# Ivordir/YALPS

Measured on AMD Instinct MI355X. Metric: fp64 pivots/sec on dense m x n tableau, higher is better.
Workload: dtype f64

## Files before the change

yalps_amd/csrc/common.cuh:

```cuda
#pragma once


constexpr int RUNNING = -1;
constexpr int SHARD_SWEEP_MISSING = 77;
constexpr int MODE_FUSED = 0, MODE_DECIDE = 1, MODE_APPLY = 2, MODE_SHARD = 3;
constexpr int SHARD_HDR = 8;
constexpr int MAX_SHARDS = 8;
constexpr int LAUNCHES_PER_GRAPH = 64;
constexpr int MAX_BLOCKS = 1024;
constexpr unsigned long long FLUSHED = 0x7FF8C0DEC0DE5EEDull;

struct alignas(16) YConst {
    int32_t height;
    int32_t check_cycles;
    int64_t hist_cap;
    int32_t *hist_leaving, *hist_entering;
    double precision, max_pivots;
};

struct alignas(16) YState {
    int32_t status;
    int32_t phase;
    int32_t bootstrap;
    int32_t la;
// ... 23 lines not shown
#ifndef YALPS_PANEL_SETS
#define YALPS_PANEL_SETS 1
#endif
constexpr int HP_SCAL = 8 + 2 * 16;
constexpr int STREAM3_MAXD = 16;
constexpr int STREAM3_PANEL_UNITS = 512;
__host__ __device__ constexpr int stream3_panel_units(int) { return STREAM3_PANEL_UNITS; }
constexpr int STREAM3_DEPTH_J16 = 16;
constexpr int DSHARD_MAXD = 16;
constexpr int DSHARD_PANEL_UNITS = 512;

struct alignas(16) Part {
    double key;
    int32_t idx;
    int32_t pad_;
};

struct Desc {
    double *mat[2];
    double *rhs[2];
    int32_t *pos, *var;
    YState *st;
    YConst *cst;
    Part *part_ratio[2];
    Part *part_rhs[2];
    int32_t w, n, pitch, hcap;
    int32_t nb;
    int32_t nshards, shard_rank, row_base;
    int32_t bounds[MAX_SHARDS + 1];
    double *rc_rows[2];
    double *rc_key[2];
    double *rc_tag[2];
    unsigned long long *rc_flag[2];
    int32_t *rc_err;
    unsigned long long *rc_verdict;
    unsigned long long *rc_rowflag;
    double *ob_park;
    int32_t *hp_xcc;
    unsigned long long *hp_flag;
    double *hp_scal;
    int32_t perm_len;
    int32_t extra;
    int32_t xl_ofs;
    double *gen_prow, *gen_scal;
    unsigned long long *sw_sync, *sw_recs;
    int32_t sw_nt;
    int32_t delay_depth;
    double *pend;
    double *obj[2];
    double *dpend, *dcolv, *dnqv, *dlav;
    DelayState *dstate;
    int32_t *cyc_verdict;
    int32_t ext_sweep;
    unsigned long long *dbg;
};
constexpr int STAMP_WORDS = 24;

struct KI {
    double k;
    int i;
};

__device__ __forceinline__ bool ki_better(double ka, int ia, double kb, int ib) {
    return ka < kb || (ka == kb && ia < ib);
}

constexpr int DPP_XOR1 = 0xB1, DPP_XOR2 = 0x4E, DPP_HALF_MIRROR = 0x141, DPP_MIRROR = 0x140;

template <int CTRL>
__device__ __forceinline__ int dpp_i32(int v) {
    return __builtin_amdgcn_update_dpp(v, v, CTRL, 0xF, 0xF, false);
}
template <int CTRL>
__device__ __forceinline__ double dpp_f64(double v) {
    const int lo = dpp_i32<CTRL>(__double2loint(v)), hi = dpp_i32<CTRL>(__double2hiint(v));
    return __hiloint2double(hi, lo);
}
__device__ __forceinline__ double row16_min(double v) {
    v = fmin(v, dpp_f64<DPP_XOR1>(v));
    v = fmin(v, dpp_f64<DPP_XOR2>(v));
    v = fmin(v, dpp_f64<DPP_HALF_MIRROR>(v));
    v = fmin(v, dpp_f64<DPP_MIRROR>(v));
    return v;
}
__device__ __forceinline__ int row16_min(int v) {
    v = min(v, dpp_i32<DPP_XOR1>(v));
    v = min(v, dpp_i32<DPP_XOR2>(v));
    v = min(v, dpp_i32<DPP_HALF_MIRROR>(v));
// ... 125 lines not shown
```

yalps_amd/csrc/resident2_kernel.cuh:

```cuda
#pragma once


__device__ __forceinline__ double min_f64_raw(double a, double b) {
    double r;
    asm("v_min_f64 %0, %1, %2" : "=v"(r) : "v"(a), "v"(b));
    return r;
}
constexpr int DPP_ROW_BCAST15 = 0x142, DPP_ROW_BCAST31 = 0x143;
template <int CTRL, int ROW_MASK>
__device__ __forceinline__ int dpp_i32_rm(int v) {
    return __builtin_amdgcn_update_dpp(v, v, CTRL, ROW_MASK, 0xF, false);
}
template <int CTRL, int ROW_MASK>
__device__ __forceinline__ double dpp_f64_rm(double v) {
    const int lo = dpp_i32_rm<CTRL, ROW_MASK>(__double2loint(v)), hi = dpp_i32_rm<CTRL, ROW_MASK>(__double2hiint(v));
    return __hiloint2double(hi, lo);
}
template <int STEPS>
__device__ __forceinline__ double rowN_min_raw(double v) {
    v = min_f64_raw(v, dpp_f64<DPP_XOR1>(v));
    if constexpr (STEPS >= 2) v = min_f64_raw(v, dpp_f64<DPP_XOR2>(v));
    if constexpr (STEPS >= 3) v = min_f64_raw(v, dpp_f64<DPP_HALF_MIRROR>(v));
    if constexpr (STEPS >= 4) v = min_f64_raw(v, dpp_f64<DPP_MIRROR>(v));
    return v;
// ... 14 lines not shown
    r.k = lane_f64(m, 63);
    const bool hit = v.k == r.k;
    const unsigned long long mask = __builtin_amdgcn_ballot_w64(hit);
    if (__popcll(mask) == 1) {
        r.i = __builtin_amdgcn_readlane(v.i, __ffsll((long long)mask) - 1);
    } else {
        int i = rowN_min<4>(hit ? v.i : INT_MAX);
        i = min(i, dpp_i32_rm<DPP_ROW_BCAST15, 0xA>(i));
        i = min(i, dpp_i32_rm<DPP_ROW_BCAST31, 0xC>(i));
        r.i = __builtin_amdgcn_readlane(i, 63);
    }
    return r;
}
template <int T>
__device__ __forceinline__ KI block_argmin2(KI v, double (*sk)[16], int (*si)[16], int slot) {
    constexpr int NW = T / 64, STEPS = NW == 16 ? 4 : NW == 8 ? 3 : NW == 4 ? 2 : 1;
    static_assert(NW == 2 || NW == 4 || NW == 8 || NW == 16, "waves per workgroup");
    v = wave_argmin2(v);
    const int lane = threadIdx.x & 63, wv = threadIdx.x >> 6;
    if (lane == 0) {
        sk[slot][wv] = v.k;
        si[slot][wv] = v.i;
    }
    __syncthreads();
    const double k = sk[slot][lane & (NW - 1)];
    const int i = si[slot][lane & (NW - 1)];
    const double km = rowN_min_raw<STEPS>(k);
    KI r;
    r.k = uniform_f64(km);
    r.i = __builtin_amdgcn_readfirstlane(rowN_min<STEPS>(k == km ? i : INT_MAX));
    return r;
}

template <int T, int J, int R>
__global__ __launch_bounds__(T) void resident2_kernel(Desc d, int parity, int chunk) {
    constexpr int SPLIT = YALPS_SPLIT_NUM * R / 4;
    constexpr unsigned FULL = (1u << (2 * J)) - 1u;
    __shared__ double sk[2][16];
    __shared__ int si[2][16];
    __shared__ double sh_cf[2][R + 2];
    __shared__ double sh_nq[R + 2];
    __shared__ double sh_raw[R + 2];
    __shared__ double sh_ck;
    __shared__ int sh_ci, sh_cg, sh_fail, sh_flag, sh_verdict, sh_pnz;
    extern __shared__ int sh_perm[];

    const int tid = threadIdx.x, NB = d.nb, b = blockIdx.x;
    const int wave = __builtin_amdgcn_readfirstlane(tid >> 6);
    const YState *Sin = d.st + parity;
    YState *Sout = d.st + (parity ^ 1);
    const YConst *C = d.cst;
    if (Sin->status != RUNNING) {
        if (b == 0 && tid == 0) state_copy(Sout, Sin);
        return;
    }
    const int h = C->height, n = d.n, pitch = d.pitch, w = d.w;
    const double precision = C->precision, max_pivots = C->max_pivots;
    const int mbuf = Sin->mbuf;
    const double *matA = d.mat[mbuf];
    const double *rhsA = d.rhs[mbuf];
    int phase = Sin->phase;
    double iter = Sin->iter;
    int64_t pivots = Sin->pivots;
    int64_t hist_len = Sin->hist_len;
    const bool check_cycles = C->check_cycles != 0;
    int slot = 0;

    int cofs[J];
#pragma unroll
    for (int j = 0; j < J; j++) {
        const int c0 = 2 * (tid + j * T);
        cofs[j] = c0 < pitch ? c0 : 0;
    }
    unsigned padmask = 0;
#pragma unroll
    for (int j = 0; j < J; j++)
#pragma unroll
        for (int k = 0; k < 2; k++)
            if (2 * (tid + j * T) + k >= n) padmask |= 1u << (2 * j + k);
    double2 x[R][J], o[J];
#pragma unroll
    for (int j = 0; j < J; j++) {
        o[j] = *reinterpret_cast<const double2 *>(matA + cofs[j]);
        if (padmask & (1u << (2 * j))) o[j].x = -INFINITY;
        if (padmask & (1u << (2 * j + 1))) o[j].y = -INFINITY;
    }
#pragma unroll
    for (int g = 0; g < R; g++) {
        const int r = b + NB * g;
        const double *mr = matA + (size_t)(r < h ? r : b) * pitch;
#pragma unroll
        for (int j = 0; j < J; j++) x[g][j] = *reinterpret_cast<const double2 *>(mr + cofs[j]);
    }
    const int my_r = b + NB * tid;
    const bool my_live = tid < R && my_r < h;
    double my_rhs = rhsA[my_live ? my_r : 0];
    if (b == 0) {
        for (int i = tid; i < d.perm_len; i += T) {
            sh_perm[i] = d.var[i];
            sh_perm[d.perm_len + i] = d.pos[i];
        }
    }
    if (tid == 0) sh_fail = 0;
    __syncthreads();

    int la = 0;
    double la_val = 0.0;
    unsigned epoch = 0;
    int cur = 0;
    auto price = [&]() __attribute__((always_inline)) {
        double best = precision;
        int bi = INT_MAX;
#pragma unroll
        for (int j = 0; j < J; j++) {
            const int c0 = 2 * (tid + j * T);
            if (o[j].x > best) {
                best = o[j].x;
                bi = c0 + 1;
            }
            if (o[j].y > best) {
                best = o[j].y;
                bi = c0 + 2;
            }
        }
        KI v = {bi == INT_MAX ? INFINITY : -best, bi};
        v = block_argmin2<T>(v, sk, si, slot);
        slot ^= 1;
        la = v.i == INT_MAX ? 0 : v.i;
        la_val = -v.k;
    };
    auto deposit_la = [&](const double2 (&pvn)[J], unsigned nzmask, bool pending) __attribute__((always_inline)) {
        const int ula = (la - 1) >> 1, ela = (la - 1) & 1, lt = ula % T, lj = ula / T;
        if (la > 0 && wave == (lt >> 6)) {
#pragma unroll
            for (int j = 0; j < J; j++)
#pragma unroll
                for (int e = 0; e < 2; e++)
                    if (2 * (tid + j * T) + e + 1 == la) {
#pragma unroll
                        for (int g = 0; g < R; g++) sh_raw[g] = e ? x[g][j].y : x[g][j].x;
                        if (pending) {
// ... 23 lines not shown
            }
            if (kind == 2 && tid < R) sh_cf[which][tid] = value;
            c = wave_argmin2(c);
            if (tid == 0) {
                sh_ck = c.k;
                sh_ci = c.i;
                sh_cg = c.i == INT_MAX ? 0 : c.i / NB;
            }
        }
        if (barrier) __syncthreads();
    };
    auto publish_flag = [&]() __attribute__((always_inline)) {
        const int par = epoch & 1;
        asm volatile("s_waitcnt vmcnt(0)" ::: "memory");
        __syncthreads();
        if (tid == 0)
            st16_sc1(reinterpret_cast<double *>(d.rc_flag[par] + 2 * b),
                     make_double2(sh_ck, __longlong_as_double((long long)(((unsigned long long)epoch << 32) | (unsigned)sh_ci))));
    };
    auto publish_stores = [&](int cg) __attribute__((always_inline)) {
        epoch++;
        double *dst = d.rc_rows[epoch & 1] + (size_t)b * pitch;
#pragma unroll
        for (int g = 0; g < R; g++) {
            if (g == cg) {
#pragma unroll
                for (int j = 0; j < J; j++) {
                    const int c0 = 2 * (tid + j * T);
                    if (c0 < pitch) st16_sc1(dst + c0, x[g][j]);
                }
            }
        }
        if (tid == cg) st_sc1(d.rc_key[epoch & 1] + b, my_rhs);
    };
    int done = 0, term = RUNNING;
    double term_result = NAN;
    bool stop = false;
#ifdef YALPS_STAMPS
    unsigned long long st_acc[20] = {}, st_last = 0, st_t0 = 0, st_r0 = 0;
#endif
    auto check = [&]() __attribute__((always_inline)) {
        if (done == chunk) {
            stop = true;
        } else if (!(iter < max_pivots)) {
            term = YALPS_CYCLED;
            stop = true;
        } else if (phase == 2 && la == 0) {
            term = YALPS_OPTIMAL;
            stop = true;
        }
    };
    const double2 no_row[J] = {};
    auto open_round = [&]() __attribute__((always_inline)) {
        double value = 0.0;
        if (phase == 2) {
            deposit_la(no_row, 0u, false);
            if (tid < R) value = sh_raw[tid];
        }
        candidate(phase, value, cur, true);
        publish_stores(__builtin_amdgcn_readfirstlane(sh_cg));
        publish_flag();
    };

    price();
    check();
    if (!stop) open_round();
#ifdef YALPS_STAMPS
    asm volatile("s_memtime %0\n\ts_memrealtime %1\n\ts_waitcnt lgkmcnt(0)" : "=s"(st_t0), "=s"(st_r0)::"memory");
    st_last = st_t0;
#endif
    while (!stop) {
        const int par = epoch & 1;
        KI c = {INFINITY, INT_MAX};
        if (tid < NB) {
            unsigned long long f = 0;
            unsigned spins = 0;
            [[maybe_unused]] unsigned long long spin_t0 = 0;
            double2 rec;
            for (;;) {
                rec = ld16_sc1_one(d.rc_flag[par] + 2 * tid);
                f = (unsigned long long)__double_as_longlong(rec.y);
                if ((unsigned)(f >> 32) == epoch) break;
                if (RESIDENT_SPIN_EXPIRED(spins, spin_t0, d.rc_err)) {
                    sh_fail = 1;
                    __hip_atomic_store(d.rc_err, 1, __ATOMIC_RELAXED, __HIP_MEMORY_SCOPE_AGENT);
                    break;
                }
                __builtin_amdgcn_s_sleep(2);
            }
            c.i = (int)(unsigned)f;
            c.k = rec.x;
#ifdef YALPS_AB_POLL_GUARD
            if (c.i != INT_MAX && (unsigned)c.i >= (unsigned)h) {
// ... 8 lines not shown
        YSTAMP(1);
        if (sh_fail) return;
        if (c.i == INT_MAX) {
            if (phase == 1) {
                phase = 2;
                iter = 0.0;
                hist_len = 0;
                check();
                if (!stop) open_round();
            } else {
                term = YALPS_UNBOUNDED;
                term_result = (double)la;
                stop = true;
            }
            YSTAMP(14);
            continue;
        }
#if defined(YALPS_AB_RETURN_GUARD) || defined(YALPS_AB_NOGUARD) || defined(YALPS_AB_POLL_GUARD)
        const int row = c.i, owner = row % NB;
#else
        const int row_in = c.i, row = (unsigned)row_in < (unsigned)h ? row_in : 0, owner = row % NB;
        if (row != row_in && tid == 0) __hip_atomic_store(d.rc_err, 1, __ATOMIC_RELAXED, __HIP_MEMORY_SCOPE_AGENT);
#endif
#ifdef YALPS_AB_RETURN_GUARD
        if ((unsigned)row >= (unsigned)h) {
            if (tid == 0) __hip_atomic_store(d.rc_err, 1, __ATOMIC_RELAXED, __HIP_MEMORY_SCOPE_AGENT);
            return;
        }
#endif
        const double *src = d.rc_rows[par] + (size_t)owner * pitch;
        double2 pv[J];
        const double rhs_row = ld_sc1(d.rc_key[par] + owner);
        double q = ld_sc1(src + (phase == 2 ? la - 1 : 0));
        ld16_sc1<J>(pv, src, cofs);
        YSTAMP(2);
        int col = la;
        double coef0 = la_val;
        if (phase == 1) {
            KI e = {INFINITY, INT_MAX};
#pragma unroll
            for (int j = 0; j < J; j++) {
                const int c0 = 2 * (tid + j * T);
#pragma unroll
                for (int k = 0; k < 2; k++) {
                    const double coefficient = elem(pv[j], k);
                    if (c0 + k < n && coefficient < -precision) {
                        const double ratio = -elem(o[j], k) / coefficient;
                        if (ratio > -INFINITY && ki_better(-ratio, c0 + k + 1, e.k, e.i)) {
                            e.k = -ratio;
                            e.i = c0 + k + 1;
                        }
                    }
                }
            }
            e = block_argmin2<T>(e, sk, si, slot);
            slot ^= 1;
            if (e.i == INT_MAX) {
                term = YALPS_INFEASIBLE;
                stop = true;
                continue;
            }
            col = e.i;
            const int ucol1 = (col - 1) >> 1, ecol1 = (col - 1) & 1;
            if (tid == ucol1 % T) {
#pragma unroll
                for (int j = 0; j < J; j++)
                    if (j == ucol1 / T) {
#pragma unroll
// ... 34 lines not shown
                __syncthreads();
                if (sh_fail) return;
                cycled = sh_verdict;
            }
            hist_len += 1;
            if (cycled) {
                term = YALPS_CYCLED;
                stop = true;
                continue;
            }
        }
        YSTAMP(3);
        const int ucol = (col - 1) >> 1, ecol = (col - 1) & 1, col_tid = ucol % T, col_j = ucol / T;
        const int col_wave = col_tid >> 6;
        double cf[R];
#pragma unroll
        for (int g = 0; g < R; g++)
            cf[g] = (T >= 512 && J * R >= 18) ? uniform_f64(sh_cf[cur][g]) : sh_cf[cur][g];
        const double my_coef = tid < R ? sh_cf[cur][tid] : 0.0;
        const int lane = tid & 63;
        const double lane_cf = sh_cf[cur][lane < R ? lane : 0];
        const unsigned long long touched = __builtin_amdgcn_ballot_w64(lane < R && b + NB * lane < h && fabs(lane_cf) > 1e-16);
        const unsigned long long live = __builtin_amdgcn_ballot_w64(lane < R && b + NB * lane < h);
        const bool all_touched = touched == live;
        unsigned nzmask = 0;
#pragma unroll
        for (int j = 0; j < J; j++) {
            const bool nzx = fabs(pv[j].x) > 1e-16, nzy = fabs(pv[j].y) > 1e-16;
            pv[j].x = nzx ? pv[j].x / q : 0.0;
            pv[j].y = nzy ? pv[j].y / q : 0.0;
            nzmask |= (nzx ? 1u : 0u) << (2 * j) | (nzy ? 1u : 0u) << (2 * j + 1);
        }
        const bool fast = __builtin_amdgcn_ballot_w64(((nzmask | padmask) & FULL) != FULL) == 0;
        const bool nz_rhs = fabs(rhs_row) > 1e-16;
        const int lslot = owner == b ? row / NB : -1;
        double my_nq = 0.0;
        if (wave == 0) {
            const double num = tid < R ? -my_coef : tid == R + 1 ? 1.0 : rhs_row;
            const double quot = num / q;
            my_nq = quot;
            if (tid < R || tid == R + 1) sh_nq[tid] = quot;
            const double rhs_q = lane_f64(quot, R + 2);
            if (my_live) {
                const double pn_rhs = nz_rhs ? rhs_q : 0.0;
                if (tid == lslot)
                    my_rhs = pn_rhs;
                else if (fabs(my_coef) > 1e-16 && nz_rhs) {
                    const double prod = my_coef * pn_rhs;
                    my_rhs = my_rhs - prod;
                }
            }
        }
        if (fabs(coef0) > 1e-16) {
            if (fast) {
#pragma unroll
                for (int j = 0; j < J; j++) {
                    const double px = coef0 * pv[j].x, py = coef0 * pv[j].y;
                    o[j].x = o[j].x - px;
                    o[j].y = o[j].y - py;
                }
            } else {
#pragma unroll
                for (int j = 0; j < J; j++) {
                    const double px = coef0 * pv[j].x, py = coef0 * pv[j].y;
                    const double nx = o[j].x - px, ny = o[j].y - py;
                    o[j].x = (nzmask & (1u << (2 * j))) ? nx : o[j].x;
                    o[j].y = (nzmask & (1u << (2 * j + 1))) ? ny : o[j].y;
                }
            }
            if (wave == col_wave) {
                if (tid == col_tid) {
                    const double nq0 = -coef0 / q;
#pragma unroll
                    for (int j = 0; j < J; j++)
                        if (j == col_j) {
                            if (ecol)
                                o[j].y = nq0;
                            else
                                o[j].x = nq0;
                        }
                }
            }
        }
        YSTAMP(5);
        iter += 1.0;
        pivots += 1;
        done += 1;
        price();
        check();
        YSTAMP(6);
        auto finish_rows = [&](unsigned long long set) __attribute__((always_inline)) {
            const unsigned long long pivbit = lslot >= 0 ? (1ull << lslot) & set : 0ull;
            const unsigned long long elim = set & touched & ~pivbit;
#pragma unroll
            for (int g = 0; g < R; g++) {
                if ((pivbit >> g) & 1u) {
#pragma unroll
                    for (int j = 0; j < J; j++) x[g][j] = pv[j];
                } else if ((elim >> g) & 1u) {
                    if (fast) {
#pragma unroll
                        for (int j = 0; j < J; j++) {
                            const double px = cf[g] * pv[j].x, py = cf[g] * pv[j].y;
                            x[g][j].x = x[g][j].x - px;
                            x[g][j].y = x[g][j].y - py;
                        }
                    } else {
#pragma unroll
                        for (int j = 0; j < J; j++) {
                            const double px = cf[g] * pv[j].x, py = cf[g] * pv[j].y;
                            const double nx = x[g][j].x - px, ny = x[g][j].y - py;
                            x[g][j].x = (nzmask & (1u << (2 * j))) ? nx : x[g][j].x;
                            x[g][j].y = (nzmask & (1u << (2 * j + 1))) ? ny : x[g][j].y;
                        }
                    }
                }
            }
            if (wave == col_wave && (elim | pivbit) != 0) {
                if (tid == col_tid) {
#pragma unroll
                    for (int g = 0; g < R; g++) {
                        if (!(((elim | pivbit) >> g) & 1u)) continue;
                        const double v = sh_nq[((pivbit >> g) & 1u) ? R + 1 : g];
#pragma unroll
                        for (int j = 0; j < J; j++)
                            if (j == col_j) {
                                if (ecol)
                                    x[g][j].y = v;
                                else
                                    x[g][j].x = v;
                            }
                    }
                }
            }
        };
        constexpr unsigned long long ONE = 1, ALL = (ONE << R) - 1, LOW = (ONE << SPLIT) - 1;
        if (!stop) {
            double value = 0.0;
            if (phase == 2) {
                deposit_la(pv, nzmask, true);
                YSTAMP(7);
                if (tid < R) {
                    value = sh_raw[tid];
                    if (tid == lslot)
                        value = la == col ? sh_nq[R + 1] : sh_raw[R];
                    else if (my_live && fabs(my_coef) > 1e-16) {
                        if (la == col)
                            value = my_nq;
                        else if (sh_pnz) {
                            const double prod = my_coef * sh_raw[R];
                            value = value - prod;
                        }
                    }
                }
            }
            if (fast && all_touched) {
                candidate(phase, value, cur ^ 1, true);
                const int cg = __builtin_amdgcn_readfirstlane(sh_cg);
                double2 cand[J];
                double ccf = 0.0;
#pragma unroll
                for (int g = 0; g < R; g++)
                    if (g == cg) {
                        ccf = cf[g];
#pragma unroll
                        for (int j = 0; j < J; j++) cand[j] = x[g][j];
                    }
                if (cg == lslot) {
#pragma unroll
                    for (int j = 0; j < J; j++) cand[j] = pv[j];
                } else {
#pragma unroll
                    for (int j = 0; j < J; j++) {
                        const double px = ccf * pv[j].x, py = ccf * pv[j].y;
                        cand[j].x = cand[j].x - px;
                        cand[j].y = cand[j].y - py;
                    }
                }
                if (wave == col_wave) {
                    if (tid == col_tid) {
                        const double v = sh_nq[cg == lslot ? R + 1 : cg];
#pragma unroll
                        for (int j = 0; j < J; j++)
                            if (j == col_j) {
                                if (ecol)
                                    cand[j].y = v;
                                else
                                    cand[j].x = v;
                            }
                    }
                }
                epoch++;
                {
                    double *dst = d.rc_rows[epoch & 1] + (size_t)b * pitch;
#pragma unroll
                    for (int j = 0; j < J; j++) {
                        const int c0 = 2 * (tid + j * T);
                        if (c0 < pitch) st16_sc1(dst + c0, cand[j]);
                    }
                    if (tid == cg) st_sc1(d.rc_key[epoch & 1] + b, my_rhs);
                }
                publish_flag();
#pragma unroll
                for (int g = 0; g < R; g++)
#pragma unroll
                    for (int j = 0; j < J; j++) {
                        const double px = cf[g] * pv[j].x, py = cf[g] * pv[j].y;
                        x[g][j].x = x[g][j].x - px;
                        x[g][j].y = x[g][j].y - py;
                    }
                if (lslot >= 0) {
#pragma unroll
                    for (int g = 0; g < R; g++)
                        if (g == lslot) {
#pragma unroll
                            for (int j = 0; j < J; j++) x[g][j] = pv[j];
                        }
                }
                if (wave == col_wave) {
                    if (tid == col_tid) {
#pragma unroll
                        for (int g = 0; g < R; g++) {
                            if (b + NB * g >= h) continue;
                            const double v = sh_nq[g == lslot ? R + 1 : g];
#pragma unroll
                            for (int j = 0; j < J; j++)
                                if (j == col_j) {
                                    if (ecol)
                                        x[g][j].y = v;
                                    else
                                        x[g][j].x = v;
                                }
                        }
                    }
                }
            } else {
                candidate(phase, value, cur ^ 1, true);
                YSTAMP(8);
                const int cg = __builtin_amdgcn_readfirstlane(sh_cg);
                finish_rows(ONE << cg);
                YSTAMP(9);
                publish_stores(cg);
                YSTAMP(10);
                if constexpr (SPLIT > 0) finish_rows(LOW & ~(ONE << cg));
                YSTAMP(11);
                publish_flag();
                YSTAMP(12);
                finish_rows(ALL & ~LOW & ~(ONE << cg));
            }
        } else {
            finish_rows(ALL);
        }
        cur ^= 1;
        if (b == 0 && tid == 0) {
            int *var = sh_perm, *pos = sh_perm + d.perm_len;
            const int leaving = var[w + row], entering = var[col];
            var[w + row] = entering;
            var[col] = leaving;
            pos[leaving] = col;
            pos[entering] = w + row;
        }
        YSTAMP(13);
    }
#ifdef YALPS_STAMPS
    if (tid == 0 && d.dbg) {
        unsigned long long t1, r1;
        asm volatile("s_memtime %0\n\ts_memrealtime %1\n\ts_waitcnt lgkmcnt(0)" : "=s"(t1), "=s"(r1)::"memory");
        unsigned long long *out = d.dbg + (size_t)b * STAMP_WORDS;
#pragma unroll
        for (int k = 0; k < 20; k++) out[k] += st_acc[k];
        out[20] += (unsigned long long)done;
        out[21] += t1 - st_t0;
        out[22] += r1 - st_r0;
    }
#endif

    double *matB = d.mat[mbuf ^ 1];
    double *rhsB = d.rhs[mbuf ^ 1];
#pragma unroll
    for (int g = 0; g < R; g++) {
        const int r = b + NB * g;
        if (r < h) {
            double *mr = matB + (size_t)r * pitch;
// ... 38 lines not shown
```

yalps_amd/csrc/yalps_hip.hip:

```cpp
#include <hip/hip_runtime.h>

#include <dlfcn.h>
#include <fcntl.h>
#include <sys/file.h>
#include <sys/stat.h>
#include <unistd.h>

#include <algorithm>
#include <atomic>
#include <chrono>
#include <climits>
#include <cmath>
#include <cstdarg>
#include <cstdint>
#include <cstdio>
#include <cstdlib>
#include <cstring>
#include <map>
#include <mutex>
#include <set>
#include <string>
#include <vector>

#include "../../include/yalps_hip.h"
// ... 180 lines not shown

int env_int(const char *name, int dflt) {
    const char *e = std::getenv(name);
    return (e && *e) ? std::atoi(e) : dflt;
}

std::string kname(const char *fmt, ...) __attribute__((format(printf, 1, 2)));
std::string kname(const char *fmt, ...) {
    char buf[96];
    va_list ap;
    va_start(ap, fmt);
    std::vsnprintf(buf, sizeof buf, fmt, ap);
    va_end(ap);
    return buf;
}

struct Kernel {
    const void *fn = nullptr;
    int lanes = 0;
    size_t lds = 0;
    std::string name;
    bool big_lds = false;
    std::string info, info_tail;
    template <class Fn> Fn as() const { return reinterpret_cast<Fn>(const_cast<void *>(fn)); }
};

struct Plan {
    int T = 0, J = 0;
    Kernel decide;
    Kernel step;
    bool wide = false;
    Kernel resident;
    bool tagged = false;
    int extra = 0, xl_ofs = 0;
    Kernel inplace[2];
    bool sweep = false;
    int sw_nt = 0;
    Kernel delayed[2];
    bool stream3 = false;
    bool ob_park = false;
    int delay_depth = 0;
    Kernel shard_step;
    bool shard_delayed = false;
    Kernel shard_sweep;
    int shard_sweep_grid = 0;
};

struct Shape {
    int width, hcap;
    int n, units;
    int pitch;
    bool too_wide;
    int T, J;
    int nb, rows_per_block;
    size_t tab_bytes;
};

Shape shape_of(int width, int hcap, int max_blocks) {
    const int n = width - 1, units = (n + 1) / 2, pitch = std::max(16, (n + 15) / 16 * 16);
    const int T = units <= 512 ? 256 : 1024;
    int J = 1;
    while (T * J < units) J *= 2;
    const bool too_wide = J > 8;
    const int nb = std::min(hcap, max_blocks);
    return {width, hcap, n, units, pitch, too_wide, T, too_wide ? 8 : J, nb, (hcap + nb - 1) / nb, sizeof(double) * (size_t)pitch * hcap};
}
// ... 6 lines not shown
        pick = &v;
        if (v.R >= (forceR ? forceR : s.rows_per_block)) break;
    }
    p.T = s.T;
    p.J = s.J;
    p.decide = Kernel{reinterpret_cast<const void *>(pick->fn), s.T, 0, kname("pivot_kernel<%d,%d,%d>", s.T, s.J, pick->R)};
    p.step = p.decide;
    p.wide = s.J >= 4 || (s.T == 1024 && s.J >= 2) || s.rows_per_block > pick->R || env_int("YALPS_HIP_WIDE", 0);
    const size_t lds = sizeof(double) * ((size_t)s.pitch + 4 * (size_t)s.rows_per_block);
    for (const WVariant &v : kWide)
        if (p.wide && v.T == s.T && v.J == s.J) p.step = Kernel{reinterpret_cast<const void *>(v.fn), s.T, lds, kname("wide_kernel<%d,%d>", s.T, s.J)};
}

void plan_resident(const Shape &s, Plan &p) {
    int best = INT_MAX, fT = 0, fJ = 0, fR = 0;
    if (const char *force = std::getenv("YALPS_HIP_RVARIANT")) std::sscanf(force, "%d,%d,%d", &fT, &fJ, &fR);
    RVariant pick{0, 0, 0, nullptr};
    const char *gen = "", *mark = "";
    size_t lds = 0;
    for (const RVariant &v : kResident) {
        if (v.T * v.J < s.units || v.R < s.rows_per_block) continue;
        if (fT && (v.T != fT || v.J != fJ || v.R != fR)) continue;
        const int regs = v.J * v.R * 1024 + v.T;
        if (regs < best) {
            best = regs;
            pick = v;
        }
    }
    if (pick.fn && env_int("YALPS_HIP_RESIDENT_GEN", 2) >= 2)
        for (const RVariant &v : kResident2)
            if (v.T == pick.T && v.J == pick.J && v.R == pick.R) {
                pick = v;
                gen = "2";
            }
    if (!pick.fn && env_int("YALPS_HIP_LDS_ROWS", 1)) {
        const int xl_ofs = (2 * (s.width + s.hcap) + 3) / 4 * 4;
        int best_extra = INT_MAX;
        for (const RVariant &v : kResidentLds) {
            const int extra = s.rows_per_block - v.R;
            if (v.T * v.J < s.units || extra < 1 || extra > XROWS) continue;
            if (fT && (v.T != fT || v.J != fJ || v.R != fR)) continue;
            const size_t bytes = sizeof(int32_t) * (size_t)xl_ofs + sizeof(double) * (size_t)extra * s.pitch;
            if (bytes > LDS_DYNAMIC_MAX || extra >= best_extra) continue;
            best_extra = extra;
            pick = v;
            lds = bytes;
            mark = ",lds";
            p.extra = extra;
            p.xl_ofs = xl_ofs;
        }
    }
    if (pick.fn && !p.extra && env_int("YALPS_HIP_TAG", 1))
        for (const RVariant &v : kResidentTag)
            if (v.T == pick.T && v.J == pick.J && v.R == pick.R) {
                pick = v;
                gen = "";
                mark = ",tag";
                p.tagged = true;
            }
    if (pick.fn)
        p.resident = Kernel{pick.fn, pick.T, lds, kname("resident%s_kernel<%d,%d,%d%s>", gen, pick.T, pick.J, pick.R, mark)};
}

void plan_inplace(const Shape &s, Plan &p) {
    const size_t rows = (size_t)s.rows_per_block;
    const size_t stream_lds = sizeof(double) * ((size_t)s.pitch + 3 * rows) + sizeof(int32_t) * rows;
    if (stream_lds <= 150 * 1024) {
        for (int check = 0; check < 2; check++)
            for (const RVariant &v : check ? kStreamCheck : kStream)
                if (v.T == s.T && v.J == s.J) p.inplace[check] = Kernel{v.fn, v.T, stream_lds, kname("stream_kernel<%d,%d%s>", v.T, v.J, check ? ",check" : "")};
    }
    const int sweep_mode = env_int("YALPS_HIP_SWEEP", 1);
    if (sweep_mode && (s.J == 8 || (s.J == 4 && (s.tab_bytes > SWEEP_BEYOND_CACHE || sweep_mode == 2)))) {
        const size_t lds = sizeof(double) * 2 * 512 * (size_t)(2 * s.J) + (4 * sizeof(double) + sizeof(int32_t)) * rows + 64;
        if (lds <= 150 * 1024) {
            int want_nt = s.tab_bytes > SWEEP_BEYOND_CACHE ? 1 : 0;
            if (const char *e = std::getenv("YALPS_HIP_SWEEP_NT")) want_nt = std::atoi(e) != 0;
            const int sT = 512, sJ = 2 * s.J;
            for (const RVariant &v : kSweep)
                if (v.T == sT && v.J == sJ && v.R == want_nt) {
                    p.inplace[0] = Kernel{v.fn, sT, lds, kname("sweep_kernel<%d,%d%s>", sT, sJ, want_nt ? ",nt" : "")};
                    p.sweep = true;
                }
            if (p.sweep) {
                p.inplace[1] = Kernel();
                for (const RVariant &v : kSweepCheck)
                    if (v.T == sT && v.J == sJ && v.R == want_nt)
                        p.inplace[1] = Kernel{v.fn, sT, lds, kname("sweep_kernel<%d,%d,check%s>", sT, sJ, want_nt ? ",nt" : "")};
                p.sw_nt = want_nt;
            }
        }
// ... 494 lines not shown
        HIP_TRY(hipMalloc(&d.gen_prow, sizeof(double) * (size_t)d.pitch));
        HIP_TRY(hipMalloc(&d.gen_scal, sizeof(double) * 4));
    }
    t->perm_cap = (width + hcap + 3) / 4 * 4;
    HIP_TRY(hipMalloc(&t->perm_block, sizeof(int32_t) * 2 * (size_t)t->perm_cap));
    d.pos = t->perm_block;
    d.var = t->perm_block + t->perm_cap;
    for (int k = 0; k < 2; k++) {
        HIP_TRY(hipMalloc(&d.part_ratio[k], sizeof(Part) * MAX_BLOCKS));
        HIP_TRY(hipMalloc(&d.part_rhs[k], sizeof(Part) * MAX_BLOCKS));
    }
    d.perm_len = t->perm_len;
    if (p.stream3) {
        HIP_TRY(hipMalloc(&d.pend, sizeof(double) * 8 * 2 * (size_t)p.delay_depth * d.pitch));
        if (p.ob_park) HIP_TRY(hipMalloc(&d.ob_park, sizeof(double) * (size_t)t->nb * d.pitch));
    }
    const bool persistent = p.resident.fn || p.inplace[0].fn;
    if (persistent) {
        for (int k = 0; k < 2; k++) {
            HIP_TRY(hipMalloc(&d.rc_rows[k], sizeof(double) * (size_t)t->nb * d.pitch));
            HIP_TRY(hipMalloc(&d.rc_key[k], sizeof(double) * ((size_t)t->nb + 8)));
        }
    }
    {
        static_assert(sizeof(YState) % 8 == 0 && sizeof(YConst) % 8 == 0, "control block layout");
        const size_t nflag = persistent ? 2 * (size_t)t->nb : 0;
        const size_t tag_row = 2 * (size_t)d.pitch + 2;
        const size_t tag_bytes = p.tagged ? sizeof(double) * 2 * (size_t)t->nb * tag_row : 0;
        const size_t sweep_bytes = p.sweep ? ((size_t)yalps_sweep_sync_bytes() + 15) / 16 * 16 + 32 * 2 * (size_t)t->nb : 0;
        const size_t hp_xcc_bytes = p.stream3 ? (sizeof(int32_t) * (size_t)t->nb + 15) / 16 * 16 : 0;
        const size_t hp_flag_bytes = p.stream3 ? sizeof(unsigned long long) * 2 * (size_t)t->nb : 0;
        const size_t hp_scal_bytes = p.stream3 ? sizeof(double) * 2 * (size_t)t->nb * HP_SCAL : 0;
        const size_t hp_bytes = hp_xcc_bytes + hp_flag_bytes + hp_scal_bytes;
        t->rc_sync_bytes = sizeof(unsigned long long) * (2 * nflag + 2) + tag_bytes + sweep_bytes + hp_bytes + 32 + 16;
        HIP_TRY(hipMalloc(&t->ctl_block, t->rc_sync_bytes + 2 * sizeof(YState) + sizeof(YConst)));
        HIP_TRY(hipMemsetAsync(t->ctl_block, 0, t->rc_sync_bytes + 2 * sizeof(YState) + sizeof(YConst), s));
        t->rc_sync = t->ctl_block;
        unsigned long long *base = static_cast<unsigned long long *>(t->ctl_block);
        d.rc_flag[0] = base;
        d.rc_flag[1] = base + nflag;
        d.rc_verdict = base + 2 * nflag;
        if (p.tagged) {
            d.rc_tag[0] = reinterpret_cast<double *>(base + 2 * nflag + 2);
            d.rc_tag[1] = d.rc_tag[0] + (size_t)t->nb * tag_row;
        }
        if (p.sweep) {
            char *sw = reinterpret_cast<char *>(base + 2 * nflag + 2) + tag_bytes;
            d.sw_sync = reinterpret_cast<unsigned long long *>(sw);
            d.sw_recs = reinterpret_cast<unsigned long long *>(sw + ((size_t)yalps_sweep_sync_bytes() + 15) / 16 * 16);
        }
        if (p.stream3) {
            char *hp = reinterpret_cast<char *>(base + 2 * nflag + 2) + tag_bytes + sweep_bytes;
            d.hp_xcc = reinterpret_cast<int32_t *>(hp);
            d.hp_flag = reinterpret_cast<unsigned long long *>(hp + hp_xcc_bytes);
            d.hp_scal = reinterpret_cast<double *>(hp + hp_xcc_bytes + hp_flag_bytes);
        }
        char *tail = static_cast<char *>(t->ctl_block) + t->rc_sync_bytes;
        d.rc_err = reinterpret_cast<int32_t *>(tail - 16);
        d.rc_rowflag = reinterpret_cast<unsigned long long *>(tail - 48);
        d.st = reinterpret_cast<YState *>(tail);
        d.cst = reinterpret_cast<YConst *>(tail + 2 * sizeof(YState));
        HIP_TRY(hipHostMalloc(reinterpret_cast<void **>(&t->host_ctl), 16 + 2 * sizeof(YState) + sizeof(YConst), hipHostMallocDefault));
    }
    HIP_TRY(hipHostMalloc(&t->host_state, sizeof(YState) * 4 + sizeof(YConst), hipHostMallocDefault));
#ifdef YALPS_STAMPS
    HIP_TRY(hipMalloc(&d.dbg, sizeof(unsigned long long) * STAMP_WORDS * MAX_BLOCKS));
    HIP_TRY(hipMemsetAsync(d.dbg, 0, sizeof(unsigned long long) * STAMP_WORDS * MAX_BLOCKS, s));
#endif
    for (int k = 0; k < 4; k++) HIP_TRY(hipEventCreateWithFlags(&t->slot_ev[k], hipEventDisableTiming));
    HIP_TRY(hipStreamSynchronize(s));
    *out = t;
    return 0;
}

int32_t yalps_tableau_create(yalps_ctx *ctx, int32_t width, int32_t hcap, yalps_tableau **out) {
    if (!ctx || !out || width < 1 || hcap < 1) return fail(YALPS_E_ARG, "yalps_tableau_create: bad argument");
    *out = nullptr;
    const int32_t rc = tableau_create_impl(ctx, width, hcap, out);
    if (rc && *out) {
        const std::string why = g_err;
        yalps_tableau_destroy(*out);
        *out = nullptr;
        g_err = why;
    }
    return rc;
}

void yalps_tableau_destroy(yalps_tableau *t) {
    if (!t) return;
    (void)hipSetDevice(t->ctx->device);
    (void)hipStreamSynchronize(t->ctx->stream);
    for (int k = 0; k < 2; k++) {
        if (t->graph_exec[k]) (void)hipGraphExecDestroy(t->graph_exec[k]);
        if (t->graph[k]) (void)hipGraphDestroy(t->graph[k]);
    }
    if (t->cut_pin) (void)hipHostFree(t->cut_pin);
    Desc &d = t->d;
    void *bufs[] = {d.mat[0], d.mat[1], d.rhs[0], d.rhs[1], t->perm_block ? nullptr : d.pos, t->perm_block ? nullptr : d.var, t->perm_block,
                    t->ctl_block ? nullptr : d.st, t->ctl_block ? nullptr : d.cst, t->ctl_block, d.rc_rows[0], d.rc_rows[1], t->perm_backup,
                    d.rc_key[0], d.rc_key[1], d.gen_prow, d.gen_scal, d.part_ratio[0], d.part_ratio[1], d.part_rhs[0], d.part_rhs[1],
                    t->hist[0], t->hist[1], t->cells, d.dbg, d.obj[0], d.pend, d.ob_park, t->dsh_block, t->cyc_block};
    for (void *p : bufs)
        if (p) (void)hipFree(p);
    if (t->host_state) (void)hipHostFree(t->host_state);
    if (t->host_ctl) (void)hipHostFree(t->host_ctl);
    if (t->pin_out) (void)hipHostFree(t->pin_out);
    for (auto &e : t->slot_ev)
        if (e) (void)hipEventDestroy(e);
    delete t;
}

int32_t yalps_tableau_height(const yalps_tableau *t) { return t ? t->height : 0; }

int32_t yalps_tableau_info(const yalps_tableau *t, char *buf, int32_t len) {
    if (!t || !buf || len < 1) return fail(YALPS_E_ARG, "yalps_tableau_info: bad argument");
    const Plan &p = t->plan;
    std::string res = "none", inp = "none", launched;
    if (p.resident.fn) res = p.resident.name + kname(" chunk=%d lds_rows=%d", RESIDENT_CHUNK, t->d.extra);
    if (p.delayed[0].fn && t->last_delayed)
        inp = (p.delayed[0].info.empty() ? p.delayed[0].name : p.delayed[0].info) + kname(" delay_depth=%d", t->d.delay_depth) + p.delayed[0].info_tail;
    else if (p.inplace[0].fn)
        inp = p.inplace[0].name;
    for (const std::string &k : t->launched) launched += (launched.empty() ? "" : "+") + k;
    const std::string str = p.shard_delayed ? p.shard_step.name + kname(",delay_depth:%d", t->d.delay_depth) : p.step.name;
    std::snprintf(buf, (size_t)len, "streaming=%s workgroups=%d resident=%s inplace=%s giveups=%lld resident_off_for=%d inplace_off_for=%d "
                  "last_path=%s last_resident_launches=%lld node_fused_runs=%lld lock_giveups=%lld decide=%s shard_sweep=%s launched=%s", str.c_str(),
                  t->nb, res.c_str(), inp.c_str(), (long long)t->giveups, t->ctx->resident ? t->ctx->resident_skip : -1,
                  t->ctx->inplace ? t->ctx->inplace_skip : -1,
                  t->last_path == 1 ? "resident" : t->last_path == 2 ? "streaming" : t->last_path == 3 ? "resident+streaming"
                  : t->last_path == 4 ? "small" : t->last_path == 8 ? "inplace" : t->last_path == 10 ? "inplace+streaming"
                  : t->last_path == 9 ? "resident+inplace" : t->last_path == 11 ? "resident+inplace+streaming"
                  : t->last_path == 16 ? "generic" : "none",
                  (long long)(t->last_path & 9 ? t->last_launches : 0), (long long)t->node_fused_runs, (long long)t->ctx->lock_giveups,
                  p.decide.name.c_str(), !p.shard_delayed ? "none" : t->d.ext_sweep ? "launch" : "inline",
                  launched.empty() ? "none" : launched.c_str());
    return 0;
}

int32_t yalps_tableau_debug_stamps(yalps_tableau *t, uint64_t *out, int32_t cap_words, int32_t reset) {
#ifdef YALPS_STAMPS
    if (!t || !t->d.dbg || (cap_words > 0 && !out)) return fail(YALPS_E_ARG, "yalps_tableau_debug_stamps: bad argument");
    HIP_TRY(hipSetDevice(t->ctx->device));
    HIP_TRY(hipStreamSynchronize(t->ctx->stream));
    const int32_t words = t->nb * STAMP_WORDS < cap_words ? t->nb * STAMP_WORDS : cap_words;
    if (words > 0) HIP_TRY(hipMemcpy(out, t->d.dbg, sizeof(uint64_t) * (size_t)words, hipMemcpyDeviceToHost));
    if (reset) HIP_TRY(hipMemset(t->d.dbg, 0, sizeof(unsigned long long) * STAMP_WORDS * MAX_BLOCKS));
    return words;
#else
    (void)t, (void)out, (void)cap_words, (void)reset;
    return fail(YALPS_E_ARG, "yalps_tableau_debug_stamps: this is not the diagnostic build (-DYALPS_STAMPS)");
#endif
// ... 1606 lines not shown
```

Baseline: 178,500.

## Speculatively publish next entering column from pivot-row owner in resident2 kernel

The block owning the pivot row now computes the next entering column (argmax of the updated objective row) speculatively and publishes it, tagged with an epoch, in a new per-block rc_next record. Other blocks load this record together with the pivot row and can skip their own pricing pass and the objective update on the critical path. This removes a full pricing reduction and a barrier from each pivot. In exchange it adds an extra spin-wait on the record, more shared state and synchronization, and a new failure path when the record never arrives.

```diff
diff --git a/yalps_amd/csrc/common.cuh b/yalps_amd/csrc/common.cuh
--- a/yalps_amd/csrc/common.cuh
+++ b/yalps_amd/csrc/common.cuh
@@ -79,6 +79,7 @@
     double *rc_key[2];
     double *rc_tag[2];
     unsigned long long *rc_flag[2];
+    unsigned long long *rc_next[2];
     int32_t *rc_err;
     unsigned long long *rc_verdict;
     unsigned long long *rc_rowflag;
@@ -101,6 +102,7 @@
     int32_t ext_sweep;
     unsigned long long *dbg;
 };
+constexpr unsigned AHEAD_NONE = 0xffffffffu;
 constexpr int STAMP_WORDS = 24;
 
 struct KI {
diff --git a/yalps_amd/csrc/resident2_kernel.cuh b/yalps_amd/csrc/resident2_kernel.cuh
--- a/yalps_amd/csrc/resident2_kernel.cuh
+++ b/yalps_amd/csrc/resident2_kernel.cuh
@@ -70,6 +70,33 @@
     return r;
 }
 
+template <int J>
+__device__ __forceinline__ void ld16_sc1_rec(double2 (&out)[J], const double *base, const int (&ofs)[J], const void *recp, double2 &rec) {
+    static_assert(J >= 1 && J <= 3, "lane units per row of the resident2_kernel shapes");
+    v2f64 t[J], r;
+#define YLD "global_load_dwordx4 %"
+    if constexpr (J == 1) {
+        asm volatile(YLD "0, %2, off sc1\n\t" YLD "1, %3, off sc1\n\ts_waitcnt vmcnt(0)"
+                     : "=&v"(r), "=&v"(t[0])
+                     : "v"(recp), "v"(base + ofs[0])
+                     : "memory");
+    } else if constexpr (J == 2) {
+        asm volatile(YLD "0, %3, off sc1\n\t" YLD "1, %4, off sc1\n\t" YLD "2, %5, off sc1\n\ts_waitcnt vmcnt(0)"
+                     : "=&v"(r), "=&v"(t[0]), "=&v"(t[1])
+                     : "v"(recp), "v"(base + ofs[0]), "v"(base + ofs[1])
+                     : "memory");
+    } else {
+        asm volatile(YLD "0, %4, off sc1\n\t" YLD "1, %5, off sc1\n\t" YLD "2, %6, off sc1\n\t" YLD "3, %7, off sc1\n\ts_waitcnt vmcnt(0)"
+                     : "=&v"(r), "=&v"(t[0]), "=&v"(t[1]), "=&v"(t[2])
+                     : "v"(recp), "v"(base + ofs[0]), "v"(base + ofs[1]), "v"(base + ofs[2])
+                     : "memory");
+    }
+#undef YLD
+    rec = make_double2(r.x, r.y);
+#pragma unroll
+    for (int j = 0; j < J; j++) out[j] = make_double2(t[j].x, t[j].y);
+}
+
 template <int T, int J, int R>
 __global__ __launch_bounds__(T) void resident2_kernel(Desc d, int parity, int chunk) {
     constexpr int SPLIT = YALPS_SPLIT_NUM * R / 4;
@@ -81,6 +108,7 @@
     __shared__ double sh_raw[R + 2];
     __shared__ double sh_ck;
     __shared__ int sh_ci, sh_cg, sh_fail, sh_flag, sh_verdict, sh_pnz;
+    __shared__ int sh_slow[2];
     extern __shared__ int sh_perm[];
 
     const int tid = threadIdx.x, NB = d.nb, b = blockIdx.x;
@@ -139,12 +167,16 @@
             sh_perm[d.perm_len + i] = d.pos[i];
         }
     }
-    if (tid == 0) sh_fail = 0;
+    if (tid == 0) {
+        sh_fail = 0;
+        sh_slow[0] = sh_slow[1] = 0;
+    }
     __syncthreads();
 
     int la = 0;
     double la_val = 0.0;
     unsigned epoch = 0;
+    const bool ahead = d.rc_next[0] != nullptr;
     int cur = 0;
     auto price = [&]() __attribute__((always_inline)) {
         double best = precision;
@@ -234,6 +266,44 @@
             }
         }
         if (tid == cg) st_sc1(d.rc_key[epoch & 1] + b, my_rhs);
+    };
+    auto publish_none = [&]() __attribute__((always_inline)) {
+        if (ahead && tid == 0)
+            st16_sc1(reinterpret_cast<double *>(d.rc_next[epoch & 1] + 2 * b),
+                     make_double2(0.0, __longlong_as_double((long long)(((unsigned long long)epoch << 32) | AHEAD_NONE))));
+    };
+    auto speculate = [&](const double2 (&cr)[J], int cg) __attribute__((always_inline)) {
+        const double qn = uniform_f64(sh_cf[cur ^ 1][cg]);
+        const bool upd = fabs(la_val) > 1e-16;
+        const double nq0 = -la_val / qn;
+        double best = precision;
+        int bi = INT_MAX;
+#pragma unroll
+        for (int j = 0; j < J; j++)
+#pragma unroll
+            for (int e = 0; e < 2; e++) {
+                const int c = 2 * (tid + j * T) + e + 1;
+                const double cv = elem(cr[j], e);
+                double ov = elem(o[j], e);
+                const bool nz = fabs(cv) > 1e-16;
+                const double pvn = nz ? cv / qn : 0.0;
+                const double prod = la_val * pvn;
+                const double nv = ov - prod;
+                if (upd) {
+                    ov = nz ? nv : ov;
+                    ov = c == la ? nq0 : ov;
+                }
+                if (ov > best) {
+                    best = ov;
+                    bi = c;
+                }
+            }
+        KI v = {bi == INT_MAX ? INFINITY : -best, bi};
+        v = block_argmin2<T>(v, sk, si, slot);
+        slot ^= 1;
+        if (tid == 0)
+            st16_sc1(reinterpret_cast<double *>(d.rc_next[epoch & 1] + 2 * b),
+                     make_double2(-v.k, __longlong_as_double((long long)(((unsigned long long)epoch << 32) | (unsigned)(v.i == INT_MAX ? 0 : v.i)))));
     };
     int done = 0, term = RUNNING;
     double term_result = NAN;
@@ -261,6 +331,7 @@
         }
         candidate(phase, value, cur, true);
         publish_stores(__builtin_amdgcn_readfirstlane(sh_cg));
+        publish_none();
         publish_flag();
     };
 
@@ -335,8 +406,38 @@
         double2 pv[J];
         const double rhs_row = ld_sc1(d.rc_key[par] + owner);
         double q = ld_sc1(src + (phase == 2 ? la - 1 : 0));
-        ld16_sc1<J>(pv, src, cofs);
-        YSTAMP(2);
+        unsigned ncol = AHEAD_NONE;
+        double nval = 0.0;
+        if (ahead) {
+            const unsigned long long *recp = d.rc_next[par] + 2 * owner;
+            double2 rec;
+            ld16_sc1_rec<J>(pv, src, cofs, recp, rec);
+            YSTAMP(2);
+            unsigned spins = 0;
+            [[maybe_unused]] unsigned long long spin_t0 = 0;
+            bool lost = false;
+            for (;;) {
+                const unsigned long long f = (unsigned long long)__double_as_longlong(rec.y);
+                if ((unsigned)__builtin_amdgcn_readfirstlane((int)(f >> 32)) == epoch) break;
+                if (__builtin_amdgcn_ballot_w64(RESIDENT_SPIN_EXPIRED(spins, spin_t0, d.rc_err)) != 0) {
+                    sh_fail = 1;
+                    __hip_atomic_store(d.rc_err, 1, __ATOMIC_RELAXED, __HIP_MEMORY_SCOPE_AGENT);
+                    lost = true;
+                    break;
+                }
+                __builtin_amdgcn_s_sleep(1);
+                rec = ld16_sc1_one(recp);
+            }
+            if (!lost) {
+                ncol = (unsigned)__builtin_amdgcn_readfirstlane((int)(unsigned)(unsigned long long)__double_as_longlong(rec.y));
+                nval = uniform_f64(rec.x);
+            }
+            YSTAMP(15);
+        } else {
+            ld16_sc1<J>(pv, src, cofs);
+            YSTAMP(2);
+        }
+        const bool have_next = ncol != AHEAD_NONE;
         int col = la;
         double coef0 = la_val;
         if (phase == 1) {
@@ -437,14 +538,16 @@
             nzmask |= (nzx ? 1u : 0u) << (2 * j) | (nzy ? 1u : 0u) << (2 * j + 1);
         }
         const bool fast = __builtin_amdgcn_ballot_w64(((nzmask | padmask) & FULL) != FULL) == 0;
+        if (!fast) sh_slow[cur] = 1;
+        if (tid == 0) sh_slow[cur ^ 1] = 0;
         const bool nz_rhs = fabs(rhs_row) > 1e-16;
         const int lslot = owner == b ? row / NB : -1;
         double my_nq = 0.0;
         if (wave == 0) {
-            const double num = tid < R ? -my_coef : tid == R + 1 ? 1.0 : rhs_row;
+            const double num = tid < R ? -my_coef : tid == R ? -coef0 : tid == R + 1 ? 1.0 : rhs_row;
             const double quot = num / q;
             my_nq = quot;
-            if (tid < R || tid == R + 1) sh_nq[tid] = quot;
+            if (tid <= R + 1) sh_nq[tid] = quot;
             const double rhs_q = lane_f64(quot, R + 2);
             if (my_live) {
                 const double pn_rhs = nz_rhs ? rhs_q : 0.0;
@@ -456,42 +559,51 @@
                 }
             }
         }
-        if (fabs(coef0) > 1e-16) {
-            if (fast) {
-#pragma unroll
-                for (int j = 0; j < J; j++) {
-                    const double px = coef0 * pv[j].x, py = coef0 * pv[j].y;
-                    o[j].x = o[j].x - px;
-                    o[j].y = o[j].y - py;
-                }
-            } else {
-#pragma unroll
-                for (int j = 0; j < J; j++) {
-                    const double px = coef0 * pv[j].x, py = coef0 * pv[j].y;
-                    const double nx = o[j].x - px, ny = o[j].y - py;
-                    o[j].x = (nzmask & (1u << (2 * j))) ? nx : o[j].x;
-                    o[j].y = (nzmask & (1u << (2 * j + 1))) ? ny : o[j].y;
-                }
-            }
-            if (wave == col_wave) {
-                if (tid == col_tid) {
-                    const double nq0 = -coef0 / q;
-#pragma unroll
-                    for (int j = 0; j < J; j++)
-                        if (j == col_j) {
-                            if (ecol)
-                                o[j].y = nq0;
-                            else
-                                o[j].x = nq0;
-                        }
-                }
-            }
-        }
+        auto update_o = [&]() __attribute__((always_inline)) {
+            if (fabs(coef0) > 1e-16) {
+                if (fast) {
+#pragma unroll
+                    for (int j = 0; j < J; j++) {
+                        const double px = coef0 * pv[j].x, py = coef0 * pv[j].y;
+                        o[j].x = o[j].x - px;
+                        o[j].y = o[j].y - py;
+                    }
+                } else {
+#pragma unroll
+                    for (int j = 0; j < J; j++) {
+                        const double px = coef0 * pv[j].x, py = coef0 * pv[j].y;
+                        const double nx = o[j].x - px, ny = o[j].y - py;
+                        o[j].x = (nzmask & (1u << (2 * j))) ? nx : o[j].x;
+                        o[j].y = (nzmask & (1u << (2 * j + 1))) ? ny : o[j].y;
+                    }
+                }
+                if (wave == col_wave) {
+                    if (tid == col_tid) {
+                        const double nq0 = -coef0 / q;
+#pragma unroll
+                        for (int j = 0; j < J; j++)
+                            if (j == col_j) {
+                                if (ecol)
+                                    o[j].y = nq0;
+                                else
+                                    o[j].x = nq0;
+                            }
+                    }
+                }
+            }
+        };
         YSTAMP(5);
         iter += 1.0;
         pivots += 1;
         done += 1;
-        price();
+        if (!have_next || !(fast && all_touched)) update_o();
+        if (have_next) {
+            la = (int)ncol;
+            la_val = nval;
+        } else {
+            price();
+            if (ahead && sh_fail) return;
+        }
         check();
         YSTAMP(6);
         auto finish_rows = [&](unsigned long long set) __attribute__((always_inline)) {
@@ -544,6 +656,7 @@
             double value = 0.0;
             if (phase == 2) {
                 deposit_la(pv, nzmask, true);
+                if (ahead && sh_fail) return;
                 YSTAMP(7);
                 if (tid < R) {
                     value = sh_raw[tid];
@@ -561,7 +674,10 @@
             }
             if (fast && all_touched) {
                 candidate(phase, value, cur ^ 1, true);
+                YSTAMP(8);
                 const int cg = __builtin_amdgcn_readfirstlane(sh_cg);
+                const bool spec = ahead && phase == 2 && __builtin_amdgcn_readfirstlane(sh_slow[cur]) == 0;
+                const bool has_cand = __builtin_amdgcn_readfirstlane(sh_ci) != INT_MAX;
                 double2 cand[J];
                 double ccf = 0.0;
 #pragma unroll
@@ -605,7 +721,33 @@
                     }
                     if (tid == cg) st_sc1(d.rc_key[epoch & 1] + b, my_rhs);
                 }
+                if (!spec) publish_none();
+                YSTAMP(10);
                 publish_flag();
+                YSTAMP(12);
+                if (have_next && fabs(coef0) > 1e-16) {
+#pragma unroll
+                    for (int j = 0; j < J; j++) {
+                        const double px = coef0 * pv[j].x, py = coef0 * pv[j].y;
+                        o[j].x = o[j].x - px;
+                        o[j].y = o[j].y - py;
+                    }
+                    if (wave == col_wave) {
+                        if (tid == col_tid) {
+                            const double nq0 = sh_nq[R];
+#pragma unroll
+                            for (int j = 0; j < J; j++)
+                                if (j == col_j) {
+                                    if (ecol)
+                                        o[j].y = nq0;
+                                    else
+                                        o[j].x = nq0;
+                                }
+                        }
+                    }
+                }
+                if (spec && has_cand) speculate(cand, cg);
+                YSTAMP(16);
 #pragma unroll
                 for (int g = 0; g < R; g++)
 #pragma unroll
@@ -649,11 +791,13 @@
                 YSTAMP(10);
                 if constexpr (SPLIT > 0) finish_rows(LOW & ~(ONE << cg));
                 YSTAMP(11);
+                publish_none();
                 publish_flag();
                 YSTAMP(12);
                 finish_rows(ALL & ~LOW & ~(ONE << cg));
             }
         } else {
+            if (have_next) __syncthreads();
             finish_rows(ALL);
         }
         cur ^= 1;
diff --git a/yalps_amd/csrc/yalps_hip.hip b/yalps_amd/csrc/yalps_hip.hip
--- a/yalps_amd/csrc/yalps_hip.hip
+++ b/yalps_amd/csrc/yalps_hip.hip
@@ -236,6 +236,7 @@
     bool wide = false;
     Kernel resident;
     bool tagged = false;
+    bool ahead = false;
     int extra = 0, xl_ofs = 0;
     Kernel inplace[2];
     bool sweep = false;
@@ -308,6 +309,7 @@
             if (v.T == pick.T && v.J == pick.J && v.R == pick.R) {
                 pick = v;
                 gen = "2";
+                p.ahead = env_int("YALPS_HIP_RESIDENT_AHEAD", 1) != 0;
             }
     if (!pick.fn && env_int("YALPS_HIP_LDS_ROWS", 1)) {
         const int xl_ofs = (2 * (s.width + s.hcap) + 3) / 4 * 4;
@@ -333,6 +335,7 @@
                 gen = "";
                 mark = ",tag";
                 p.tagged = true;
+                p.ahead = false;
             }
     if (pick.fn)
         p.resident = Kernel{pick.fn, pick.T, lds, kname("resident%s_kernel<%d,%d,%d%s>", gen, pick.T, pick.J, pick.R, mark)};
@@ -893,7 +896,8 @@
         const size_t hp_flag_bytes = p.stream3 ? sizeof(unsigned long long) * 2 * (size_t)t->nb : 0;
         const size_t hp_scal_bytes = p.stream3 ? sizeof(double) * 2 * (size_t)t->nb * HP_SCAL : 0;
         const size_t hp_bytes = hp_xcc_bytes + hp_flag_bytes + hp_scal_bytes;
-        t->rc_sync_bytes = sizeof(unsigned long long) * (2 * nflag + 2) + tag_bytes + sweep_bytes + hp_bytes + 32 + 16;
+        const size_t next_bytes = p.ahead ? sizeof(unsigned long long) * 2 * nflag : 0;
+        t->rc_sync_bytes = sizeof(unsigned long long) * (2 * nflag + 2) + tag_bytes + sweep_bytes + hp_bytes + next_bytes + 32 + 16;
         HIP_TRY(hipMalloc(&t->ctl_block, t->rc_sync_bytes + 2 * sizeof(YState) + sizeof(YConst)));
         HIP_TRY(hipMemsetAsync(t->ctl_block, 0, t->rc_sync_bytes + 2 * sizeof(YState) + sizeof(YConst), s));
         t->rc_sync = t->ctl_block;
@@ -915,6 +919,10 @@
             d.hp_xcc = reinterpret_cast<int32_t *>(hp);
             d.hp_flag = reinterpret_cast<unsigned long long *>(hp + hp_xcc_bytes);
             d.hp_scal = reinterpret_cast<double *>(hp + hp_xcc_bytes + hp_flag_bytes);
+        }
+        if (p.ahead) {
+            d.rc_next[0] = reinterpret_cast<unsigned long long *>(reinterpret_cast<char *>(base + 2 * nflag + 2) + tag_bytes + sweep_bytes + hp_bytes);
+            d.rc_next[1] = d.rc_next[0] + nflag;
         }
         char *tail = static_cast<char *>(t->ctl_block) + t->rc_sync_bytes;
         d.rc_err = reinterpret_cast<int32_t *>(tail - 16);
@@ -977,7 +985,7 @@
     if (!t || !buf || len < 1) return fail(YALPS_E_ARG, "yalps_tableau_info: bad argument");
     const Plan &p = t->plan;
     std::string res = "none", inp = "none", launched;
-    if (p.resident.fn) res = p.resident.name + kname(" chunk=%d lds_rows=%d", RESIDENT_CHUNK, t->d.extra);
+    if (p.resident.fn) res = p.resident.name + kname(" chunk=%d lds_rows=%d ahead=%d", RESIDENT_CHUNK, t->d.extra, p.ahead ? 1 : 0);
     if (p.delayed[0].fn && t->last_delayed)
         inp = (p.delayed[0].info.empty() ? p.delayed[0].name : p.delayed[0].info) + kname(" delay_depth=%d", t->d.delay_depth) + p.delayed[0].info_tail;
     else if (p.inplace[0].fn)
```

Result: slower. 155,300 (-13.0%).
